# amaas/stanford-ctc

Hardware: AMD Instinct MI355X
Metric: audio frames/sec (CTC fwd-bwd + BRNN grad) at T=1000, L=5, H=1824, |Sigma|=33 (higher is better)
Workload: dtype f32; 1 GPU; WSJ-shape cfg-3: T=1000 A=33 5x1824 BRNN (temporalLayer 3, inputDim 483) U=100, minibatch 32 per GPU, one costAndGrad per step; utterances_per_gpu=32, parallelism=single-gpu

## Files before the change

### stanford-ctc_amd/csrc/recurrent.hip

```cpp
#include <algorithm>
#include <atomic>
#include <map>
#include <mutex>
#include <utility>
#include <vector>

#include <dirent.h>
#include <errno.h>
#include <fcntl.h>
#include <string.h>
#include <string>
#include <type_traits>
#include <sys/stat.h>
#include <sys/file.h>
#include <time.h>
#include <unistd.h>

#include "common.h"
#include "recurrent.h"
#include "xlane.h"

namespace sctc {

typedef void (*RecKernel)(RecArgs);
// ... 365 lines not shown
    const int base = nch >> 2, rem = nch & 3;
    const int cnt = base + (wave < rem ? 1 : 0);
    const int c_beg = wave * base + min(wave, rem);
    float4* Wl = lds4 + (size_t)wave * NLDS * 64;
    float4* red = lds4 + (size_t)4 * NLDS * 64;

    auto load_w = [&](int c) {
        const float* W = p.W[g];
        float4 v;
        if (!p.transpose) {
            v = *reinterpret_cast<const float4*>(W + (int64_t)(row0 + uj) * p.ldw + 16 * c + 4 * kq);
        } else {
            const float* col = W + (int64_t)(16 * c + 4 * kq) * p.ldw + row0 + uj;
            v.x = col[0];
            v.y = col[p.ldw];
            v.z = col[2 * p.ldw];
            v.w = col[3 * p.ldw];
        }
        return v;
    };
    float4 wreg[NREG > 0 ? NREG : 1];
#pragma unroll
    for (int u = 0; u < NREG; ++u) wreg[u] = load_w(c_beg + min(u, cnt - 1));
#pragma unroll 4
    for (int u = NREG; u < NCQ; ++u) Wl[(u - NREG) * 64 + lane] = load_w(c_beg + min(u, cnt - 1));
    __syncthreads();

    const bool desc = p.descending[g] != 0;
    const float* pre = p.pre[g];
    const float* act = p.act[g];
    float* out = p.out[g];
    const int64_t ld = p.ld;
    const float hi = p.max_act > 0.f ? p.max_act : INFINITY;
    unsigned* flags = p.counters + 32 + chain * 128 * REC_FLAG_STRIDE;
    unsigned* err = p.counters + 2;
    const unsigned chunk_stride = (unsigned)p.n_xrows * 64u;
    float* xg = p.xbuf + (size_t)g * p.n_xrows * Hp;
    const __amdgpu_buffer_rsrc_t xrsrc = __builtin_amdgcn_make_buffer_rsrc(
        xg, 0, (int)((size_t)p.n_xrows * Hp * sizeof(float)), 0x00020000);

    const int ub = tile * 16 + uj;
    const int uT = ub < p.B ? p.T_b[ub] : 0;
    const int Tchain = tile * 16 < p.B ? p.T_b[tile * 16] : 0;
    const int tile_T = lane_order_steps(uT, tile, p.b_off, p.variant);

    const int dbg_sel = (p.debug && chain == 0 && tid == 0) ? (wg == 0 ? 0 : (wg == nwg - 1 ? 1 : -1)) : -1;
    auto stamp = [&](int j, int k) {
        if (dbg_sel >= 0 && j >= 64 && j < 80)
            p.debug[(dbg_sel * 16 + (j - 64)) * 8 + k] = (unsigned)clock64();
        if (p.debug && tid == 0 && j == 70) {
            p.debug[REC_DEBUG_ALL_OFF + blockIdx.x * 8 + k] = (unsigned)wall_clock64();
            if (k == 0) p.debug[REC_DEBUG_ALL_OFF + blockIdx.x * 8 + 7] = 1u + (unsigned)chain;
#ifdef SCTC_REC_WHERE
            if (k == 0)
                p.debug[REC_DEBUG_ALL_OFF + blockIdx.x * 8 + 6] =
                    ((__builtin_amdgcn_s_getreg(20 | (0 << 6) | ((4 - 1) << 11)) & 0xf) << 16) |
                    ((__builtin_amdgcn_s_getreg(4 | (0 << 6) | ((32 - 1) << 11)) >> 8) & 0xff);
#endif
        }
    };

    if ((p.variant == 5 && g == 0) || (p.variant == 6 && tile == 0) || (p.variant == 7 && ((g ^ tile) & 1) == 0))
        __builtin_amdgcn_s_setprio(3);
    int rb_next = uT > 0 ? p.rowbase[desc ? uT - 1 : 0] : 0;
    int xb_next = p.xbase[0], xb_cur = 0;
    for (int j = 0; j < Tchain; ++j) {
        stamp(j, 0);
        f32x4 acc[4];
#pragma unroll
        for (int q = 0; q < 4; ++q) acc[q] = {0.f, 0.f, 0.f, 0.f};
        const bool active = j < uT;
        const int xb_prev = xb_cur;
        const int rb = rb_next;
        xb_cur = xb_next;
        {
            const int jn = min(j + 1, Tchain - 1);
            const int tn = desc ? uT - 1 - jn : jn;
            rb_next = p.rowbase[min(max(tn, 0), p.Tmax - 1)];
            xb_next = p.xbase[jn];
        }
        const int64_t orow = active ? (int64_t)rb + p.b_off + ub : 0;
        const unsigned xrow = active ? (unsigned)xb_cur + (unsigned)ub : 0u;
        const unsigned prow = (active && j > 0) ? (unsigned)xb_prev + (unsigned)ub : 0u;
        unsigned xin = prow * 64u + (unsigned)kq * 16u;
        unsigned xout = xrow * 64u + (unsigned)kq * 16u;
        if (j > 0 && j <= tile_T && active) xin = ((unsigned)xb_prev + (unsigned)tile * 16u) * 64u + (unsigned)lane * 16u;
        if (j < tile_T) xout = ((unsigned)xb_cur + (unsigned)tile * 16u) * 64u + (unsigned)lane * 16u;
        float4 pre4 = make_float4(0.f, 0.f, 0.f, 0.f), act4 = pre4;
        if (wave == 0 && active) {
            pre4 = *reinterpret_cast<const float4*>(pre + orow * ld + row0 + 4 * kq);
            if (act) act4 = *reinterpret_cast<const float4*>(act + orow * ld + row0 + 4 * kq);
        }

        if (j > 0) {
            wait_all(flags, nwg, (unsigned)j, err, p.poll_delay);
            stamp(j, 1);
            float4 x[NCQ];
#pragma unroll
            for (int u = 0; u < NCQ; ++u) {
                x[u] = ld_x(xrsrc, xin, (unsigned)(c_beg + min(u, cnt - 1)) * chunk_stride);
                __builtin_amdgcn_sched_barrier(0);
                __builtin_amdgcn_s_sleep(1);
                __builtin_amdgcn_sched_barrier(0);
            }
            __builtin_amdgcn_sched_barrier(0);
#pragma unroll
            for (int u = 0; u < NCQ; ++u) {
                if (u < NCQ - 1 || cnt == NCQ) {
                    const float4 a = u < NREG ? wreg[u < NREG ? u : 0] : Wl[(u - NREG) * 64 + lane];
                    SCTC_MFMA4(acc, a, x[u])
                }
            }
            if (p.debug) {
                asm volatile("" : "+v"(acc[0]), "+v"(acc[1]), "+v"(acc[2]), "+v"(acc[3]));
                stamp(j, 2);
            }
            if (wave != 0) {
                const f32x4 s = (acc[0] + acc[1]) + (acc[2] + acc[3]);
                red[(wave - 1) * 64 + lane] = make_float4(s[0], s[1], s[2], s[3]);
            }
            __syncthreads();
            stamp(j, 3);
        }

        if (wave == 0 && active) {
            float4 s = make_float4(0.f, 0.f, 0.f, 0.f);
            if (j > 0) {
                const float4 r1 = red[lane], r2 = red[64 + lane], r3 = red[128 + lane];
                const f32x4 q = (acc[0] + acc[1]) + (acc[2] + acc[3]);
                s = make_float4((q[0] + r1.x) + (r2.x + r3.x), (q[1] + r1.y) + (r2.y + r3.y),
                                (q[2] + r1.z) + (r2.z + r3.z), (q[3] + r1.w) + (r2.w + r3.w));
            }
            const float4 o = step_result(pre4, s, act4, act != nullptr, hi);
            *reinterpret_cast<float4*>(out + orow * ld + row0 + 4 * kq) = o;
            st_x(xrsrc, xout, (unsigned)wg * chunk_stride, o, sync_mode);
        }
        stamp(j, 4);
        if (j + 1 < Tchain) publish_step(flags + wg * REC_FLAG_STRIDE, (unsigned)(j + 1), sync_mode);
        stamp(j, 5);
    }
}

template <int... I, class F>
__device__ __forceinline__ void static_for_seq(std::integer_sequence<int, I...>, F&& f)
{
    (f(std::integral_constant<int, I>()), ...);
}
template <int N, class F>
__device__ __forceinline__ void static_for(F&& f)
{
    static_for_seq(std::make_integer_sequence<int, N>(), static_cast<F&&>(f));
}

template <int NCQ, int NREGF, int NT, int NBAT, int R, int PUB, int PB>
__global__ __launch_bounds__(256, 1) void brnn_recurrent_t_kernel(RecArgs p)
{
    extern __shared__ __attribute__((aligned(16))) float4 lds4[];
    constexpr int NFR = 2 * NCQ;
    constexpr int NLDSF = NFR - NREGF;
    constexpr int XB = (NCQ + NBAT - 1) / NBAT;
    constexpr int NC = 2 * NT;
    static_assert(NC <= 4, "one result per wave");
    static_assert(NBAT % R == 0 && NBAT >= 2 * R && R >= 2, "ring");
    static_assert((NBAT - 1) * XB < NCQ, "no empty batch");
    static_assert(PUB >= 0 && PUB + 2 <= PB && PB <= NBAT - R + 1 && PB >= 1,
                  "the flag is published (behind batch PUB) before the next phase's flags are polled (in front of batch PB - 1) and "
                  "seen (in front of batch PB), and that before the next phase's first exchange loads (batch NBAT - R + 1)");
    const int tid = threadIdx.x, lane = tid & 63;
    const int wave = __builtin_amdgcn_readfirstlane(tid >> 6);
    const int Hp = p.Hp, nch = Hp >> 4, nprod = Hp >> 5;
    const int combo = blockIdx.x & 3, ublk = blockIdx.x >> 2;
    const int g = combo & 1, half = combo >> 1;
    const int row0 = ublk * 32;
    const int uj = lane & 15, kq = lane >> 4;
    const int sync_mode = p.sync_mode;
    const int base = nch >> 2, rem = nch & 3;
    const int cnt = base + (wave < rem ? 1 : 0);
    const int c_beg = wave * base + min(wave, rem);
    float4* Wl = lds4 + (size_t)wave * NLDSF * 64;
    float4* red = lds4 + (size_t)4 * NLDSF * 64;

    auto load_w = [&](int c, int ug) {
        const float* W = p.W[g];
        const int r = row0 + 16 * ug + uj;
        float4 v;
        if (!p.transpose) {
            v = *reinterpret_cast<const float4*>(W + (int64_t)r * p.ldw + 16 * c + 4 * kq);
        } else {
            const float* col = W + (int64_t)(16 * c + 4 * kq) * p.ldw + r;
            v.x = col[0];
            v.y = col[p.ldw];
            v.z = col[2 * p.ldw];
            v.w = col[3 * p.ldw];
        }
        return v;
    };
    float4 wreg[NREGF > 0 ? NREGF : 1];
    auto load_w0 = [&](int f) {
        const float4 w = load_w(c_beg + min(f >> 1, cnt - 1), f & 1);
        return (f >> 1) < cnt ? w : make_float4(0.f, 0.f, 0.f, 0.f);
    };
#pragma unroll
    for (int f = 0; f < NREGF; ++f) {
        const float4 w = load_w0(f);
        asm("v_accvgpr_write_b32 %0, %1" : "=a"(wreg[f].x) : "v"(w.x));
        asm("v_accvgpr_write_b32 %0, %1" : "=a"(wreg[f].y) : "v"(w.y));
        asm("v_accvgpr_write_b32 %0, %1" : "=a"(wreg[f].z) : "v"(w.z));
        asm("v_accvgpr_write_b32 %0, %1" : "=a"(wreg[f].w) : "v"(w.w));
    }
#pragma unroll 4
    for (int f = NREGF; f < NFR; ++f) Wl[(f - NREGF) * 64 + lane] = load_w0(f);
    __syncthreads();

    const bool desc = p.descending[g] != 0;
    const float* pre = p.pre[g];
    const float* act = p.act[g];
    const float* act_or_pre = act ? act : pre;
    float* out = p.out[g];
    const int64_t ld = p.ld;
    const float hi = p.max_act > 0.f ? p.max_act : INFINITY;
    unsigned* err = p.counters + 2;
    const unsigned chunk_stride = (unsigned)p.n_xrows * 64u;
    float* xg = p.xbuf + (size_t)g * p.n_xrows * Hp;
    const __amdgpu_buffer_rsrc_t xrsrc = __builtin_amdgcn_make_buffer_rsrc(
        xg, 0, (int)((size_t)p.n_xrows * Hp * sizeof(float)), 0x00020000);

    struct Sub {
        int ub[NT], uT[NT], tile_T[NT];
        unsigned trow[NT];
        int T;
        unsigned* flags;
        int rb_next[NT];
        unsigned xb_next, xb_cur;
    };
    auto init_sub = [&](Sub& S, int sub) {
#pragma unroll
        for (int i = 0; i < NT; ++i) {
            const int tile = (i * 2 + sub) * 2 + half;
            S.trow[i] = (unsigned)tile * 16u;
            S.ub[i] = tile * 16 + uj;
            S.uT[i] = S.ub[i] < p.B ? p.T_b[S.ub[i]] : 0;
            S.tile_T[i] = lane_order_steps(S.uT[i], tile, p.b_off, p.variant);
            S.rb_next[i] = S.uT[i] > 0 ? p.rowbase[desc ? S.uT[i] - 1 : 0] : 0;
        }
        S.T = __builtin_amdgcn_readfirstlane((int)S.trow[0] < p.B ? p.T_b[S.trow[0]] : 0);
        S.flags = p.counters + 32 + (size_t)((combo * 2 + sub) * 64) * REC_FLAG_STRIDE;
        S.xb_next = (unsigned)p.xbase[0];
        S.xb_cur = 0;
    };
    int vzero;
    asm volatile("v_mov_b32 %0, 0" : "=v"(vzero));
    Sub A, Bc;
    init_sub(A, 0);
    init_sub(Bc, 1);

    const int dbg_sel = (p.debug && combo == 0 && tid == 0) ? (ublk == 0 ? 0 : (ublk == nprod - 1 ? 1 : -1)) : -1;
    unsigned* dbg_lds = reinterpret_cast<unsigned*>(red + (size_t)2 * NC * 3 * 64);
#if defined(SCTC_T_STAMPS) || defined(SCTC_T_STAMP_CHUNKS)
    auto stamp = [&](int sub, int j, int k) {
        if (dbg_sel >= 0 && j >= 64 && j < 72)
            dbg_lds[((j - 64) * 2 + sub) * 8 + k] = (unsigned)wall_clock64();
    };
#else
    auto stamp = [&](int, int, int) {};
    (void)dbg_lds;
#endif
#ifdef SCTC_T_STAMP_CHUNKS
    unsigned* dbg_fine = dbg_lds + 16 * 8;
    auto stamp_chunk = [&](int sub, int j, int c) {
        if (dbg_sel >= 0 && j >= 64 && j < 68 && c < 32)
            dbg_fine[((j - 64) * 2 + sub) * 32 + c] = (unsigned)wall_clock64();
    };
#else
    auto stamp_chunk = [&](int, int, int) {};
#endif

    float4 x[R][XB][NT];

    auto xin_of = [&](const Sub& S, int j, unsigned xb_prev, unsigned (&xin)[NT]) {
#pragma unroll
        for (int i = 0; i < NT; ++i) {
            const bool active = j < S.uT[i];
            const unsigned prow = (active && j > 0) ? xb_prev + (unsigned)S.ub[i] : 0u;
            xin[i] = prow * 64u + (unsigned)kq * 16u;
            if (j > 0 && j <= S.tile_T[i] && active)
                xin[i] = (xb_prev + S.trow[i]) * 64u + (unsigned)lane * 16u;
            if (p.variant == 49) xin[i] = (unsigned)lane * 16u;
        }
    };
    auto issue_part = [&](const unsigned (&xin)[NT], auto bi_c, auto lo_c, auto hi_c) {
        constexpr int bi = decltype(bi_c)::value, lo = decltype(lo_c)::value, hi_ = decltype(hi_c)::value;
#pragma unroll
        for (int u = lo; u < hi_; ++u) {
            const int cu = bi * XB + u;
            if (cu < NCQ) {
#pragma unroll
                for (int i = 0; i < NT; ++i)
                    x[bi % R][u][i] = ld_x(xrsrc, xin[i], (unsigned)(c_beg + min(cu, cnt - 1)) * chunk_stride);
            }
        }
    };
    auto issue_batch = [&](const unsigned (&xin)[NT], auto bi_c) {
        issue_part(xin, bi_c, std::integral_constant<int, 0>(), std::integral_constant<int, XB>());
    };
    const __amdgpu_buffer_rsrc_t frsrc = __builtin_amdgcn_make_buffer_rsrc(
        p.counters, 0, (int)(REC_COUNTER_WORDS * sizeof(unsigned)), 0x00020000);
    const unsigned flane = (unsigned)min(lane, nprod - 1) * (REC_FLAG_STRIDE * 4u);
    auto flags_off = [&](const unsigned* fl) -> unsigned { return (unsigned)((fl - p.counters) * 4); };
    auto poll_issue = [&](unsigned fl_off) -> u32x4 {
        return __builtin_amdgcn_raw_buffer_load_b128(frsrc, flane, fl_off, 16 );
    };
    auto poll_min = [&](const u32x4& v) -> unsigned {
        unsigned f = v[0];
#pragma unroll
        for (int c = 1; c < NC; ++c) f = min(f, v[c]);
        return f;
    };
    auto wait_flags = [&](unsigned fl_off, unsigned f, unsigned target) {
        if (__all(f >= target)) return;
        const unsigned long long t0 = wall_clock64();
        unsigned spins = 0;
        for (;;) {
            __builtin_amdgcn_s_sleep(1);
            asm volatile("" ::: "memory");
            f = poll_min(poll_issue(fl_off));
            if (__all(f >= target)) break;
            if ((++spins & 255u) == 0) {
                if (spin_expired(err, t0, lane)) break;
            }
        }
    };
    auto prologue = [&](const Sub& S, int j) {
        first_poll_delay(p.poll_delay);
        wait_flags(flags_off(S.flags), poll_min(poll_issue(flags_off(S.flags))), (unsigned)j);
        unsigned xin[NT];
        xin_of(S, j, S.xb_cur, xin);
        static_for<R - 1>([&](auto b) { issue_batch(xin, b); });
    };

    struct Epi {
        bool pending, zero;
        bool lane_active;
        int parity;
        f32x4 mine;
        float4 pre4, act4, r0, r1, r2, s, o;
        int64_t out_off;
        unsigned xo, xchunk;
        unsigned* flag;
        unsigned val;
    };
    Epi E;
    E.pending = false;
    auto epi_barrier = [&](const Epi& e) {
        if (e.pending && !e.zero) {
            asm volatile("s_waitcnt lgkmcnt(0)" ::: "memory");
            __builtin_amdgcn_s_barrier();
            asm volatile("" ::: "memory");
        }
    };
    auto epi_read = [&](Epi& e) {
        if (e.pending && !e.zero && wave < NC) {
            const float4* r = red + (size_t)((e.parity * NC + wave) * 3) * 64 + lane;
            e.r0 = r[0];
            e.r1 = r[64];
            e.r2 = r[128];
        }
    };
    auto epi_sum = [&](Epi& e) {
        e.s = make_float4(0.f, 0.f, 0.f, 0.f);
        if (e.pending && wave < NC && !e.zero) {
            const float4 m = make_float4(e.mine[0], e.mine[1], e.mine[2], e.mine[3]);
            float4 p0 = m, p1 = e.r0, p2 = e.r1, p3 = e.r2;
            if (wave == 1) { p0 = e.r0; p1 = m; }
            if (wave == 2) { p0 = e.r0; p1 = e.r1; p2 = m; }
            if (wave == 3) { p0 = e.r0; p1 = e.r1; p2 = e.r2; p3 = m; }
            e.s = make_float4((p0.x + p1.x) + (p2.x + p3.x), (p0.y + p1.y) + (p2.y + p3.y),
                              (p0.z + p1.z) + (p2.z + p3.z), (p0.w + p1.w) + (p2.w + p3.w));
        }
    };
    auto epi_result = [&](Epi& e) {
        if (e.pending && wave < NC) e.o = step_result(e.pre4, e.s, e.act4, act != nullptr, hi);
    };
    auto epi_stores = [&](const Epi& e) {
        if (e.pending && wave < NC && e.lane_active) {
            *reinterpret_cast<float4*>(out + e.out_off) = e.o;
            st_x(xrsrc, e.xo, e.xchunk, e.o, sync_mode);
        }
    };
    auto epi_store = [&](Epi& e) {
        epi_sum(e);
        epi_result(e);
        epi_stores(e);
    };
    auto epi_publish = [&](Epi& e, auto n_after_c) {
        constexpr int n_after = decltype(n_after_c)::value;
        if (e.pending) {
            if (wave < NC) {
                asm volatile("s_waitcnt vmcnt(%0)" ::"n"(n_after) : "memory");
                if (lane == 0) {
                    if (sync_mode == 0) {
                        __builtin_amdgcn_fence(__ATOMIC_RELEASE, "agent");
                        asm volatile("s_waitcnt vmcnt(0)" ::: "memory");
                    }
                    __hip_atomic_store(e.flag, e.val, __ATOMIC_RELAXED, __HIP_MEMORY_SCOPE_AGENT);
                }
            }
            e.pending = false;
        }
    };
    auto flush = [&](Epi& e) {
        epi_barrier(e);
        epi_read(e);
        epi_store(e);
        epi_publish(e, std::integral_constant<int, 0>());
    };

    int phase_no = 0;
    auto phase = [&](Sub& S, int sub, int j, bool pre_next, const Sub& N, int jn, auto first_c) {
        constexpr bool FIRST = decltype(first_c)::value;
        stamp(sub, j, 0);
        stamp_chunk(sub, j, 0);
        auto late_loads = [&](Epi& en) {
            const int jn2 = min(j + 1, S.T - 1);
            S.xb_next = (unsigned)p.xbase[jn2 + vzero];
#pragma unroll
            for (int i = 0; i < NT; ++i) {
                const int tn = desc ? S.uT[i] - 1 - jn2 : jn2;
                S.rb_next[i] = p.rowbase[min(max(tn, 0), p.Tmax - 1)];
            }
            en.pre4 = *reinterpret_cast<const float4*>(pre + en.out_off);
            en.act4 = *reinterpret_cast<const float4*>(act_or_pre + en.out_off);
        };
        unsigned xin[NT];
        Epi En;
        auto setup = [&]() {
        const unsigned xb_prev = S.xb_cur, xb_cur = S.xb_next;
        S.xb_cur = xb_cur;
        int rb[NT];
#pragma unroll
        for (int i = 0; i < NT; ++i) rb[i] = S.rb_next[i];
        xin_of(S, j, xb_prev, xin);
        En.pending = true;
        En.zero = FIRST;
        En.parity = phase_no & 1;
        En.lane_active = false;
        En.out_off = 0;
        En.xo = 0;
        En.xchunk = (unsigned)(2 * ublk + (wave & 1)) * chunk_stride;
        En.flag = S.flags + ublk * REC_FLAG_STRIDE + wave;
        En.val = (unsigned)(j + 1);
#pragma unroll
        for (int i = 0; i < NT; ++i) {
            if ((wave >> 1) == i && wave < NC) {
                const bool active = j < S.uT[i];
                const int64_t orow = active ? (int64_t)rb[i] + p.b_off + S.ub[i] : 0;
                const unsigned xrow = active ? xb_cur + (unsigned)S.ub[i] : 0u;
                En.xo = xrow * 64u + (unsigned)kq * 16u;
                if (j < S.tile_T[i]) En.xo = (xb_cur + S.trow[i]) * 64u + (unsigned)lane * 16u;
                En.lane_active = active;
                En.out_off = orow * ld + row0 + 16 * (wave & 1) + 4 * kq;
            }
        }
        };
        if constexpr (FIRST) { setup(); late_loads(En); }
        f32x4 acc[2][NT][4];
#pragma unroll
        for (int ug = 0; ug < 2; ++ug)
#pragma unroll
            for (int i = 0; i < NT; ++i)
#pragma unroll
                for (int q = 0; q < 4; ++q) acc[ug][i][q] = {0.f, 0.f, 0.f, 0.f};

        constexpr int WA = 2;
        float4 aq[WA + 1];
        auto prefetch_a = [&](auto G_c) {
            constexpr int G = decltype(G_c)::value, cu = G / NC, f = 2 * cu + ((G % NC) & 1);
            if constexpr (cu < NCQ && f >= NREGF) aq[G % (WA + 1)] = Wl[(f - NREGF) * 64 + lane];
        };
        auto mfma_group = [&](auto bi_c, auto u_c, auto g_c) {
            constexpr int bi = decltype(bi_c)::value, u = decltype(u_c)::value, cu = bi * XB + u;
            constexpr int gi = decltype(g_c)::value >> 1, ug = decltype(g_c)::value & 1;
            constexpr int G = cu * NC + decltype(g_c)::value;
            prefetch_a(std::integral_constant<int, G + WA>());
            if constexpr (cu < NCQ) {
                constexpr int f = 2 * cu + ug;
                float4 a;
                if constexpr (f < NREGF) a = wreg[f]; else a = aq[G % (WA + 1)];
                SCTC_MFMA4(acc[ug][gi], a, x[bi % R][u][gi])
            }
        };
        auto mfma_chunk = [&](auto bi_c, auto u_c) {
            static_for<NC>([&](auto g_c) { mfma_group(bi_c, u_c, g_c); });
        };
        if constexpr (!FIRST) {
            const unsigned nfl_off = flags_off(N.flags);
            u32x4 fl = {0u, 0u, 0u, 0u};
            unsigned xin_n[NT];
#pragma unroll
            for (int i = 0; i < NT; ++i) xin_n[i] = (unsigned)kq * 16u;
            auto issue_one = [&](const unsigned (&xs)[NT], auto bi_c, auto l_c) {
                constexpr int bi = decltype(bi_c)::value, l = decltype(l_c)::value, u = l / NT, i = l % NT, cu = bi * XB + u;
                if constexpr (cu < NCQ)
                    x[bi % R][u][i] = ld_x(xrsrc, xs[i], (unsigned)(c_beg + min(cu, cnt - 1)) * chunk_stride);
            };
            auto park = [&](auto c_c) {
                constexpr int c = decltype(c_c)::value;
                float4* rp = red + (size_t)(En.parity * NC * 3) * 64 + lane;
                const f32x4 s = (acc[c & 1][c >> 1][0] + acc[c & 1][c >> 1][1]) + (acc[c & 1][c >> 1][2] + acc[c & 1][c >> 1][3]);
                if (wave == c) En.mine = s;
                else rp[(c * 3 + (wave < c ? wave : wave - 1)) * 64] = make_float4(s[0], s[1], s[2], s[3]);
            };
            static_for<WA>([&](auto G_c) { prefetch_a(G_c); });
            static_for<NBAT>([&](auto b_c) {
                constexpr int b = decltype(b_c)::value;
                constexpr int nb = b + R - 1;
                constexpr int XBb = (b + 1) * XB <= NCQ ? XB : NCQ - b * XB, NG = XBb * NC;
                constexpr int NL = XB * NT;
#define SCTC_T_SLOT(piece) (NC - 1 + (piece) < NG - 1 ? NC - 1 + (piece) : NG - 1)
                if constexpr (b == PB - 1) {
                    fl = poll_issue(nfl_off);
                    __builtin_amdgcn_sched_barrier(0);
                }
                if constexpr (b == PB) {
                    if (pre_next) {
                        wait_flags(nfl_off, poll_min(fl), (unsigned)jn);
                        xin_of(N, jn, N.xb_cur, xin_n);
                    }
                    __builtin_amdgcn_sched_barrier(0);
                }
                static_for<NG>([&](auto s_c) {
                    constexpr int s = decltype(s_c)::value;
                    mfma_group(b_c, std::integral_constant<int, s / NC>(), std::integral_constant<int, s % NC>());
                    __builtin_amdgcn_sched_barrier(0);
                    if constexpr (b == 0 && s == 0) { setup(); __builtin_amdgcn_sched_barrier(0); }
                    if constexpr (b * XB + s / NC == NCQ - 1 && s % NC >= 1) {
                        park(std::integral_constant<int, s % NC - 1>());
                        __builtin_amdgcn_sched_barrier(0);
                    }
                    if constexpr (s % NC == NC - 1) stamp_chunk(sub, j, 1 + b * XB + s / NC);
                    if constexpr (b == 0) {
                        if constexpr (s % NC == NC - 1 && s / NC < 5) stamp(sub, j, 1 + s / NC);
                        if constexpr (s == SCTC_T_SLOT(0)) { epi_barrier(E); __builtin_amdgcn_sched_barrier(0); }
                        if constexpr (s == SCTC_T_SLOT(1)) { epi_read(E); __builtin_amdgcn_sched_barrier(0); }
                        if constexpr (s == SCTC_T_SLOT(2)) { epi_sum(E); __builtin_amdgcn_sched_barrier(0); }
                        if constexpr (s == SCTC_T_SLOT(3)) { epi_result(E); __builtin_amdgcn_sched_barrier(0); }
                        if constexpr (s == SCTC_T_SLOT(4)) { epi_stores(E); __builtin_amdgcn_sched_barrier(0); }
                    }
                    static_for<NL>([&](auto l_c) {
                        constexpr int l = decltype(l_c)::value, raw = b == 0 ? SCTC_T_SLOT(5) + l : l * NG / NL;
                        if constexpr ((raw < NG - 1 ? raw : NG - 1) == s) {
                            if constexpr (nb < NBAT) issue_one(xin, std::integral_constant<int, nb>(), l_c);
                            else issue_one(xin_n, std::integral_constant<int, nb - NBAT>(), l_c);
                        }
                    });
                    __builtin_amdgcn_sched_barrier(0);
                });
                if constexpr (b == NBAT - 1) {
                    asm volatile("" : "+v"(S.xb_next));
#pragma unroll
                    for (int i = 0; i < NT; ++i) asm volatile("" : "+v"(S.rb_next[i]));
                    asm volatile("" : "+v"(En.pre4.x), "+v"(En.pre4.y), "+v"(En.pre4.z), "+v"(En.pre4.w));
                    asm volatile("" : "+v"(En.act4.x), "+v"(En.act4.y), "+v"(En.act4.z), "+v"(En.act4.w));
                    __builtin_amdgcn_sched_barrier(0);
                }
                if constexpr (b == PUB) {
                    constexpr int first = (R - 1) * XB, end = (R + PUB) * XB < NCQ ? (R + PUB) * XB : NCQ;
                    epi_publish(E, std::integral_constant<int, NT * (end - first)>());
                    __builtin_amdgcn_sched_barrier(0);
                    late_loads(En);
                    __builtin_amdgcn_sched_barrier(0);
                    stamp(sub, j, 6);
                }
            });
            stamp(sub, j, 7);
            park(std::integral_constant<int, NC - 1>());
        } else {
            En.mine = {0.f, 0.f, 0.f, 0.f};
        }
        E = En;
        ++phase_no;
    };

    if (A.T > 0) { phase(A, 0, 0, false, A, 0, std::true_type()); flush(E); }
    if (Bc.T > 0) { phase(Bc, 1, 0, false, Bc, 0, std::true_type()); flush(E); }
    Sub cur = A, nxt = Bc;
    int jc = 1, jn = 1, subc = 0;
    if (jc < cur.T) prologue(cur, jc);
    while (jc < cur.T) {
        const bool pre_next = jn < nxt.T;
        phase(cur, subc, jc, pre_next, nxt, jn, std::false_type());
        ++jc;
        if (pre_next) {
            const Sub t = cur;
            cur = nxt;
            nxt = t;
            const int tj = jc;
            jc = jn;
            jn = tj;
            subc ^= 1;
        } else {
            flush(E);
            if (jc < cur.T) prologue(cur, jc);
        }
    }
#if defined(SCTC_T_STAMPS) || defined(SCTC_T_STAMP_CHUNKS)
    if (dbg_sel >= 0) {
        for (int i = 0; i < 16 * 8; ++i) p.debug[dbg_sel * 16 * 8 + i] = dbg_lds[i];
#ifdef SCTC_T_STAMP_CHUNKS
        for (int i = 0; i < 8 * 32; ++i) p.debug[REC_DEBUG_ALL_OFF + dbg_sel * 8 * 32 + i] = dbg_fine[i];
#endif
    }
#endif
}

#ifdef SCTC_REC_EXPERIMENTS
#include "recurrent_experiments_q8.inc"
#endif

static constexpr unsigned XSENT = 0xffffffffu;

template <int NK, int SB>
__global__ __launch_bounds__(256, 1) void brnn_recurrent_s_kernel(RecArgs p)
{
    extern __shared__ __attribute__((aligned(16))) float4 lds4[];
    float* xs = reinterpret_cast<float*>(lds4);
    const int tid = threadIdx.x, lane = tid & 63;
    const int wave = __builtin_amdgcn_readfirstlane(tid >> 6);
    const int g = blockIdx.x & 1, wg = blockIdx.x >> 1;
    const int Hp = p.Hp;
    const int rg = tid >> 5, ks = tid & 31;
    const int row0 = wg * 16 + 2 * rg;
    const bool owner = ks == 31;

    float w0[NK], w1[NK];
    {
        const float* W = p.W[g];
#pragma unroll
        for (int i = 0; i < NK; ++i) {
            const int k = 32 * i + ks;
            if (!p.transpose) {
                w0[i] = W[(int64_t)row0 * p.ldw + k];
                w1[i] = W[(int64_t)(row0 + 1) * p.ldw + k];
            } else {
                w0[i] = W[(int64_t)k * p.ldw + row0];
                w1[i] = W[(int64_t)k * p.ldw + row0 + 1];
            }
        }
    }
    const bool desc = p.descending[g] != 0;
    const float* pre = p.pre[g];
    const float* act = p.act[g];
    float* out = p.out[g];
    const int64_t ld = p.ld;
    const float hi = p.max_act > 0.f ? p.max_act : INFINITY;
    unsigned* err = p.counters + 2;
    float* xg = p.xbuf + (size_t)g * p.n_xrows * Hp;
    const __amdgpu_buffer_rsrc_t xrsrc = __builtin_amdgcn_make_buffer_rsrc(
        xg, 0, (int)((size_t)p.n_xrows * Hp * sizeof(float)), 0x00020000);
    int Tb[SB];
#pragma unroll
    for (int b = 0; b < SB; ++b) Tb[b] = b < p.B ? p.T_b[b] : 0;
// ... 668 lines not shown

static int read_error_word(const RecArgs& a, hipStream_t stream, unsigned* e)
{
    *e = 0;
    SCTC_HIP_TRY(hipMemcpyAsync(e, a.counters + 2, sizeof(unsigned), hipMemcpyDeviceToHost, stream));
    SCTC_HIP_TRY(hipStreamSynchronize(stream));
    return SCTC_OK;
}

static int launch_persistent(RecKernel k, int grid, size_t smem, int max_per_cu, size_t sentinel_bytes,
                             const RecArgs& a, const LaunchCtx& cx, bool* done, int threads = 256)
{
    *done = false;
    int per_cu = 0;
    SCTC_TRY(prepare_kernel(k, threads, smem, max_per_cu, cx.dev, &per_cu));
    if (per_cu < 1 || (int64_t)per_cu * cx.cus < grid) return SCTC_OK;
    const int need_cus = (grid + per_cu - 1) / per_cu;
    if (sentinel_bytes)
        SCTC_HIP_TRY(hipMemsetAsync(a.xbuf, 0xFF, sentinel_bytes, cx.stream));
    if (!recurrent_shared_device_mode() && !g_shared_hard.load(std::memory_order_relaxed) && g_users.due(cx.dev)) {
        const int n = g_users.count(cx.dev);
        if (n > 1) {
            recurrent_set_shared_device_mode(1);
            fprintf(stderr, "sctc: %d processes run persistent kernels on this GPU: shared-device mode on "
                            "(their launches take turns under /dev/shm/sctc_gpu_*.lock)\n", n);
        }
    }
    if (recurrent_shared_device_mode()) {
        SCTC_HIP_TRY(hipStreamSynchronize(cx.stream));
        LeaseGuard lease(cx.dev);
        if (!lease.locked) return SCTC_OK;
        hipLaunchKernelGGL(k, dim3(grid), dim3(threads), smem, cx.stream, a);
        SCTC_HIP_TRY(hipGetLastError());
        unsigned e = 0;
        SCTC_TRY(read_error_word(a, cx.stream, &e));
        *done = true;
        if (cx.path) *cx.path = REC_PATH_PERSISTENT_LEASED;
        if (e != 0)
            return set_error(SCTC_ERR_TIMEOUT, "recurrent kernel: a persistent launch under the device lease gave "
                             "up waiting for its peers (%d workgroups not co-resident)", grid);
        return SCTC_OK;
    }
    SCTC_TRY(g_gate.admit_and_launch(cx.dev, cx.stream, need_cus, cx.cus, [&]() {
        hipLaunchKernelGGL(k, dim3(grid), dim3(threads), smem, cx.stream, a);
        return hipGetLastError();
    }));
    *done = true;
    if (cx.path) *cx.path = REC_PATH_PERSISTENT;
    return SCTC_OK;
}

static int launch_recurrent_one(const RecArgs& a, const LaunchCtx& cx)
{
    const int nwg = a.Hp / 16;
    const int ntiles = (a.B + 15) / 16;
    hipStream_t stream = cx.stream;
    bool done = false;
    SCTC_HIP_TRY(hipMemsetAsync(a.counters + 32, 0, (REC_COUNTER_WORDS - 32) * sizeof(unsigned), stream));
    if (a.variant == 3 || 2 * nwg > cx.cus) {
        if (cx.path) *cx.path = REC_PATH_FALLBACK;
        return launch_fallback(a, stream);
    }
    if ((!a.prec16 || a.B <= 5) && (a.B > Q1_MIN_B - 1 || a.variant == 44) && a.B <= 16 && a.variant != 1 && a.variant != 42 && a.variant != 43 &&
        2 * nwg <= cx.cus) {
        RecKernel qk = nullptr;
        int ncq = 0, nreg = 0;
        switch (nwg) {
            case 32:  qk = brnn_recurrent_q_kernel<8, 0>;   ncq = 8;  nreg = 0;  break;
            case 64:  qk = brnn_recurrent_q_kernel<16, 0>;  ncq = 16; nreg = 0;  break;
            case 114: qk = brnn_recurrent_q_kernel<29, 10>; ncq = 29; nreg = 10; break;
            case 128: qk = brnn_recurrent_q_kernel<32, 13>; ncq = 32; nreg = 13; break;
            default: break;
        }
        if (qk) {
            RecArgs b = a;
            b.linear_map = 1;
            if (b.variant == 44) b.variant = 0;
            const size_t smem = sizeof(float4) * ((size_t)4 * (ncq - nreg) * 64 + 3 * 64);
            SCTC_TRY(launch_persistent(qk, 2 * nwg, smem, 2, 0, b, cx, &done));
            if (done) return SCTC_OK;
        }
    }
    if ((a.B <= 5 || (a.B <= 8 && a.variant == 43)) && a.variant != 1) {
        RecKernel sk = nullptr;
        const bool s4 = a.B <= 4;
        switch (a.Hp / 32) {
            case 16: sk = s4 ? brnn_recurrent_s_kernel<16, 4> : brnn_recurrent_s_kernel<16, 8>; break;
            case 32: sk = s4 ? brnn_recurrent_s_kernel<32, 4> : brnn_recurrent_s_kernel<32, 8>; break;
            case 57: sk = s4 ? brnn_recurrent_s_kernel<57, 4> : brnn_recurrent_s_kernel<57, 8>; break;
            case 64: sk = s4 ? brnn_recurrent_s_kernel<64, 4> : brnn_recurrent_s_kernel<64, 8>; break;
            default: break;
        }
        if (sk) {
            const size_t smem = sizeof(float) * 2 * (s4 ? 4 : 8) * a.Hp;
            SCTC_TRY(launch_persistent(sk, 2 * nwg, smem, 2, (size_t)2 * a.n_xrows * a.Hp * sizeof(float), a, cx, &done));
            if (done) return SCTC_OK;
        }
    }
    if (a.prec16 && a.B > 5 && a.B <= 16 && a.variant != 1) {
        RecKernel hk = nullptr;
        const bool bf = a.transpose != 0;
        const int nch = a.Hp / 32;
        switch ((nch + 3) / 4) {
            case 4:  if (nch == 16) hk = bf ? brnn_recurrent_mh_kernel<4, true>  : brnn_recurrent_mh_kernel<4, false>;  break;
            case 8:  if (nch == 32) hk = bf ? brnn_recurrent_mh_kernel<8, true>  : brnn_recurrent_mh_kernel<8, false>;  break;
            case 15: if (nch == 57) hk = bf ? brnn_recurrent_mh_kernel<15, true> : brnn_recurrent_mh_kernel<15, false>; break;
            case 16: if (nch == 64) hk = bf ? brnn_recurrent_mh_kernel<16, true> : brnn_recurrent_mh_kernel<16, false>; break;
            default: break;
        }
        const size_t smem = (((size_t)16 * (a.Hp + 8) * 2 + 15) / 16) * 16 + 3 * 64 * sizeof(float4);
        if (hk && smem <= 160 * 1024) {
            SCTC_TRY(launch_persistent(hk, 2 * nwg, smem, 1, (size_t)2 * a.n_xrows * a.Hp * 2, a, cx, &done));
            if (done) return SCTC_OK;
        }
    }
#ifdef SCTC_REC_EXPERIMENTS
    if (a.B > 5 && a.B <= 16 && a.variant != 1) {
        RecKernel mk = nullptr;
        switch ((nwg + 3) / 4) {
            case 8:  if (nwg == 32)  mk = brnn_recurrent_m_kernel<8>;  break;
            case 16: if (nwg == 64)  mk = brnn_recurrent_m_kernel<16>; break;
            case 29: if (nwg == 114) mk = brnn_recurrent_m_kernel<29>; break;
            case 32: if (nwg == 128) mk = brnn_recurrent_m_kernel<32>; break;
            default: break;
        }
        const size_t smem = sizeof(float) * ((size_t)16 * (a.Hp + 4) + 3 * 256);
        if (mk && smem <= 160 * 1024) {
            SCTC_TRY(launch_persistent(mk, 2 * nwg, smem, 1, (size_t)2 * a.n_xrows * a.Hp * sizeof(float), a, cx, &done));
            if (done) return SCTC_OK;
        }
    }
#endif
#ifdef SCTC_REC_EXPERIMENTS
    const int q8_variant = (a.variant >= 8 && a.variant < 40) ? a.variant : (a.variant == 0 ? REC_Q8_DEFAULT : 0);
    if (ntiles == 2 && q8_variant >= 8) {
        RecKernel k8 = nullptr;
        switch (nwg) {
            case 32:  k8 = brnn_recurrent_q8_kernel<8>;  break;
            case 64:  k8 = brnn_recurrent_q8_kernel<16>; break;
            case 114: k8 = brnn_recurrent_q8_kernel<29>; break;
            case 128: k8 = brnn_recurrent_q8_kernel<32>; break;
            default: break;
        }
        const int grid = 8 * ((nwg + 3) / 4);
        const size_t smem = sizeof(float4) * ((size_t)nwg * 64 + 6 * 64) + sizeof(unsigned) * Q8_SYNC_WORDS;
        if (k8 && grid <= cx.cus && smem <= 160 * 1024) {
            RecArgs b = a;
            b.variant = q8_variant;
            SCTC_TRY(launch_persistent(k8, grid, smem, 1, 0, b, cx, &done, 512));
            if (done) return SCTC_OK;
        }
    }
#endif
    if (ntiles == 2 && a.variant != 1 && 4 * nwg <= 2 * cx.cus && (4 * nwg) % 8 == 0) {
        RecKernel qk = nullptr;
        int ncq = 0, nreg = 0;
        switch (nwg) {
            case 32:  qk = brnn_recurrent_q_kernel<8, 0>;   ncq = 8;  nreg = 0;  break;
            case 64:  qk = brnn_recurrent_q_kernel<16, 0>;  ncq = 16; nreg = 0;  break;
            case 114: qk = brnn_recurrent_q_kernel<29, 10>; ncq = 29; nreg = 10; break;
            case 128: qk = brnn_recurrent_q_kernel<32, 13>; ncq = 32; nreg = 13; break;
            default: break;
        }
        if (qk) {
            const size_t smem = sizeof(float4) * ((size_t)4 * (ncq - nreg) * 64 + 3 * 64);
            SCTC_TRY(launch_persistent(qk, 4 * nwg, smem, 2, 0, a, cx, &done));
            if (done) return SCTC_OK;
        }
    }
    if (ntiles > 2 && a.variant != 1 && a.variant != 40 && a.variant != 47 && 4 * (a.Hp / 32) <= cx.cus &&
        (a.Hp >= 1824 || a.variant == 50)) {
        RecKernel tk = nullptr;
        const bool one = ntiles <= 4;
        int nldsf = 0;
        static const int tcfg = getenv("SCTC_REC_TCFG") ? atoi(getenv("SCTC_REC_TCFG")) : 0;
        switch (nwg) {
            case 32:  tk = one ? brnn_recurrent_t_kernel<8, 0, 1, 4, 2, 0, 3>  : brnn_recurrent_t_kernel<8, 0, 2, 4, 2, 0, 3>;  nldsf = 16; break;
            case 64:  tk = one ? brnn_recurrent_t_kernel<16, 0, 1, 4, 2, 1, 3> : brnn_recurrent_t_kernel<16, 0, 2, 4, 2, 1, 3>; nldsf = 32; break;
            case 114:
                nldsf = 33;
                if (one) tk = tcfg == 1 ? brnn_recurrent_t_kernel<29, 25, 1, 6, 3, 1, 4> : tcfg == 2 ? brnn_recurrent_t_kernel<29, 25, 1, 8, 2, 1, 7>
                              : brnn_recurrent_t_kernel<29, 25, 1, 8, 4, 1, 5>;
                else tk = tcfg == 1 ? brnn_recurrent_t_kernel<29, 25, 2, 8, 4, 1, 5> : tcfg == 2 ? brnn_recurrent_t_kernel<29, 25, 2, 8, 2, 1, 7>
                          : brnn_recurrent_t_kernel<29, 25, 2, 6, 3, 1, 4>;
                break;
            case 128:
                nldsf = 33;
                if (one) tk = tcfg == 1 ? brnn_recurrent_t_kernel<32, 31, 1, 6, 3, 1, 4> : brnn_recurrent_t_kernel<32, 31, 1, 8, 4, 1, 5>;
                else tk = tcfg == 1 ? brnn_recurrent_t_kernel<32, 31, 2, 6, 3, 1, 4> : brnn_recurrent_t_kernel<32, 31, 2, 8, 4, 1, 5>;
                break;
            default: break;
        }
        if (tk) {
            const size_t smem = sizeof(float4) * 64 * ((size_t)4 * nldsf + 2 * 3 * (one ? 2 : 4)) + (16 * 8 + 8 * 32) * sizeof(unsigned);
            SCTC_TRY(launch_persistent(tk, 4 * (a.Hp / 32), smem, 1, 0, a, cx, &done));
            if (done) return SCTC_OK;
        }
    }
    const int ntw = ntiles <= 2 ? 1 : (ntiles <= 4 ? 2 : 4);
    const size_t smem = sizeof(float4) * ((size_t)nwg * 64 + 2 * ntw * 64);
    if (smem <= 160 * 1024) {
        const bool pipe = a.variant != 40;
        RecKernel kern = ntw == 1 ? pick_kernel<1>(nwg / 2, false)
                         : (ntw == 2 ? pick_kernel<2>(nwg / 2, pipe) : pick_kernel<4>(nwg / 2, pipe));
        SCTC_TRY(launch_persistent(kern, 2 * nwg, smem, 1, 0, a, cx, &done));
        if (done) return SCTC_OK;
    }
    if (cx.path) *cx.path = REC_PATH_FALLBACK;
    return launch_fallback(a, stream);
}

int recurrent_clear_error(unsigned* counters, hipStream_t stream)
{
    SCTC_HIP_TRY(hipMemsetAsync(counters, 0, 32 * sizeof(unsigned), stream));
    return SCTC_OK;
}

int launch_recurrent(const RecArgs& a_in, hipStream_t stream, int* path)
{
    RecArgs a = a_in;
    if (a.poll_delay < 0) a.poll_delay = a.Hp > 1024 ? 5 : 0;
    char why[128];
    if (!recurrent_supported(a.Hp, a.B, why, sizeof(why)))
        return set_error(SCTC_ERR_ARG, "recurrent kernel: %s", why);
    if (a.Tmax <= 0 || a.B <= 0) return SCTC_OK;
    if ((size_t)a.n_xrows * a.Hp * sizeof(float) >= ((size_t)1 << 31))
        return set_error(SCTC_ERR_ARG, "recurrent kernel: %d exchange rows x %d units exceed the "
                         "2 GiB buffer addressing", a.n_xrows, a.Hp);
    LaunchCtx cx;
    cx.stream = stream;
    cx.path = path;
    cx.dev = 0;
    cx.cus = 0;
    SCTC_HIP_TRY(hipGetDevice(&cx.dev));
    SCTC_HIP_TRY(hipDeviceGetAttribute(&cx.cus, hipDeviceAttributeMultiprocessorCount, cx.dev));
    constexpr int MAXB = 128;
    for (int b0 = 0; b0 < a_in.B;) {
        int nb = std::min(MAXB, a_in.B - b0);
        const bool tiled = ((a.variant == 0 && (a.Hp == 1824 || a.Hp == 2048)) || (a.variant == 50 && (a.Hp == 512 || a.Hp == 1024 || a.Hp == 1824 || a.Hp == 2048))) &&
                           !a.prec16 && 4 * (a.Hp / 32) <= cx.cus;
        if (tiled) {
            if (nb > 64 && nb <= 96) nb = 64;
        } else {
            if (nb > 32 && nb <= 48 && a.variant == 0 && !a.prec16) nb = 32;
            else if (nb > 64 && nb <= 80 && a.variant == 0 && !a.prec16) nb = 64;
        }
        RecArgs c = a;
        c.b_off = a_in.b_off + b0;
        c.T_b = a_in.T_b + b0;
        c.B = nb;
        if (a_in.T_host) c.Tmax = std::min(a_in.Tmax, (int)a_in.T_host[b0]);
        if (c.variant == 45) c.variant = 0;
        SCTC_TRY(launch_recurrent_one(c, cx));
        b0 += nb;
    }
    return SCTC_OK;
}

}
```

Measured before the change: 763,400 frames/s.

## Add 16-unit-per-block variant of transposed recurrent kernel for two-tile case

Generalizes the transposed recurrent kernel with a UG parameter so each workgroup can own 16 hidden units instead of 32. This doubles the number of producer blocks, widens the flag polling to two flags per lane, and remaps flag slots for blocks beyond 64. A new dispatch path for the two-tile fp32 case launches this variant ahead of the older q kernel, with all weights held in registers by default. The aim is to spread the serial recurrence over more CUs and cut per-block matmul work per step, at the cost of more cross-block synchronisation and flag traffic per timestep.

```diff
diff --git a/stanford-ctc_amd/csrc/recurrent.hip b/stanford-ctc_amd/csrc/recurrent.hip
--- a/stanford-ctc_amd/csrc/recurrent.hip
+++ b/stanford-ctc_amd/csrc/recurrent.hip
@@ -541,15 +541,17 @@
     static_for_seq(std::make_integer_sequence<int, N>(), static_cast<F&&>(f));
 }
 
-template <int NCQ, int NREGF, int NT, int NBAT, int R, int PUB, int PB>
+template <int NCQ, int NREGF, int NT, int NBAT, int R, int PUB, int PB, int UG = 2>
 __global__ __launch_bounds__(256, 1) void brnn_recurrent_t_kernel(RecArgs p)
 {
     extern __shared__ __attribute__((aligned(16))) float4 lds4[];
-    constexpr int NFR = 2 * NCQ;
+    constexpr int NFR = UG * NCQ;
     constexpr int NLDSF = NFR - NREGF;
     constexpr int XB = (NCQ + NBAT - 1) / NBAT;
-    constexpr int NC = 2 * NT;
-    static_assert(NC <= 4, "one result per wave");
+    constexpr int NC = UG * NT;
+    constexpr int NPL = UG == 1 ? 2 : 1;
+    static_assert(UG == 1 || UG == 2, "16 or 32 units per block");
+    static_assert(NC <= 4 && NPL * NC <= 4, "one result per wave, one 16-byte flag load per lane");
     static_assert(NBAT % R == 0 && NBAT >= 2 * R && R >= 2, "ring");
     static_assert((NBAT - 1) * XB < NCQ, "no empty batch");
     static_assert(PUB >= 0 && PUB + 2 <= PB && PB <= NBAT - R + 1 && PB >= 1,
@@ -557,10 +559,10 @@
                   "seen (in front of batch PB), and that before the next phase's first exchange loads (batch NBAT - R + 1)");
     const int tid = threadIdx.x, lane = tid & 63;
     const int wave = __builtin_amdgcn_readfirstlane(tid >> 6);
-    const int Hp = p.Hp, nch = Hp >> 4, nprod = Hp >> 5;
-    const int combo = blockIdx.x & 3, ublk = blockIdx.x >> 2;
+    const int Hp = p.Hp, nch = Hp >> 4, nprod = nch / UG;
+    const int combo = blockIdx.x & (2 * UG - 1), ublk = blockIdx.x / (2 * UG);
     const int g = combo & 1, half = combo >> 1;
-    const int row0 = ublk * 32;
+    const int row0 = ublk * 16 * UG;
     const int uj = lane & 15, kq = lane >> 4;
     const int sync_mode = p.sync_mode;
     const int base = nch >> 2, rem = nch & 3;
@@ -586,8 +588,8 @@
     };
     float4 wreg[NREGF > 0 ? NREGF : 1];
     auto load_w0 = [&](int f) {
-        const float4 w = load_w(c_beg + min(f >> 1, cnt - 1), f & 1);
-        return (f >> 1) < cnt ? w : make_float4(0.f, 0.f, 0.f, 0.f);
+        const float4 w = load_w(c_beg + min(f / UG, cnt - 1), f % UG);
+        return (f / UG) < cnt ? w : make_float4(0.f, 0.f, 0.f, 0.f);
     };
 #pragma unroll
     for (int f = 0; f < NREGF; ++f) {
@@ -625,7 +627,7 @@
     auto init_sub = [&](Sub& S, int sub) {
 #pragma unroll
         for (int i = 0; i < NT; ++i) {
-            const int tile = (i * 2 + sub) * 2 + half;
+            const int tile = (i * 2 + sub) * UG + half;
             S.trow[i] = (unsigned)tile * 16u;
             S.ub[i] = tile * 16 + uj;
             S.uT[i] = S.ub[i] < p.B ? p.T_b[S.ub[i]] : 0;
@@ -703,6 +705,11 @@
         unsigned f = v[0];
 #pragma unroll
         for (int c = 1; c < NC; ++c) f = min(f, v[c]);
+        if constexpr (NPL == 2) {
+            const bool second = lane + 64 < nprod;
+#pragma unroll
+            for (int c = 0; c < NC; ++c) f = second ? min(f, v[NC + c]) : f;
+        }
         return f;
     };
     auto wait_flags = [&](unsigned fl_off, unsigned f, unsigned target) {
@@ -835,26 +842,26 @@
         En.lane_active = false;
         En.out_off = 0;
         En.xo = 0;
-        En.xchunk = (unsigned)(2 * ublk + (wave & 1)) * chunk_stride;
-        En.flag = S.flags + ublk * REC_FLAG_STRIDE + wave;
+        En.xchunk = (unsigned)(UG * ublk + wave % UG) * chunk_stride;
+        En.flag = S.flags + (ublk & 63) * REC_FLAG_STRIDE + (ublk >> 6) * NC + wave;
         En.val = (unsigned)(j + 1);
 #pragma unroll
         for (int i = 0; i < NT; ++i) {
-            if ((wave >> 1) == i && wave < NC) {
+            if (wave / UG == i && wave < NC) {
                 const bool active = j < S.uT[i];
                 const int64_t orow = active ? (int64_t)rb[i] + p.b_off + S.ub[i] : 0;
                 const unsigned xrow = active ? xb_cur + (unsigned)S.ub[i] : 0u;
                 En.xo = xrow * 64u + (unsigned)kq * 16u;
                 if (j < S.tile_T[i]) En.xo = (xb_cur + S.trow[i]) * 64u + (unsigned)lane * 16u;
                 En.lane_active = active;
-                En.out_off = orow * ld + row0 + 16 * (wave & 1) + 4 * kq;
+                En.out_off = orow * ld + row0 + 16 * (wave % UG) + 4 * kq;
             }
         }
         };
         if constexpr (FIRST) { setup(); late_loads(En); }
-        f32x4 acc[2][NT][4];
-#pragma unroll
-        for (int ug = 0; ug < 2; ++ug)
+        f32x4 acc[UG][NT][4];
+#pragma unroll
+        for (int ug = 0; ug < UG; ++ug)
 #pragma unroll
             for (int i = 0; i < NT; ++i)
 #pragma unroll
@@ -863,16 +870,16 @@
         constexpr int WA = 2;
         float4 aq[WA + 1];
         auto prefetch_a = [&](auto G_c) {
-            constexpr int G = decltype(G_c)::value, cu = G / NC, f = 2 * cu + ((G % NC) & 1);
+            constexpr int G = decltype(G_c)::value, cu = G / NC, f = UG * cu + (G % NC) % UG;
             if constexpr (cu < NCQ && f >= NREGF) aq[G % (WA + 1)] = Wl[(f - NREGF) * 64 + lane];
         };
         auto mfma_group = [&](auto bi_c, auto u_c, auto g_c) {
             constexpr int bi = decltype(bi_c)::value, u = decltype(u_c)::value, cu = bi * XB + u;
-            constexpr int gi = decltype(g_c)::value >> 1, ug = decltype(g_c)::value & 1;
+            constexpr int gi = decltype(g_c)::value / UG, ug = decltype(g_c)::value % UG;
             constexpr int G = cu * NC + decltype(g_c)::value;
             prefetch_a(std::integral_constant<int, G + WA>());
             if constexpr (cu < NCQ) {
-                constexpr int f = 2 * cu + ug;
+                constexpr int f = UG * cu + ug;
                 float4 a;
                 if constexpr (f < NREGF) a = wreg[f]; else a = aq[G % (WA + 1)];
                 SCTC_MFMA4(acc[ug][gi], a, x[bi % R][u][gi])
@@ -895,7 +902,7 @@
             auto park = [&](auto c_c) {
                 constexpr int c = decltype(c_c)::value;
                 float4* rp = red + (size_t)(En.parity * NC * 3) * 64 + lane;
-                const f32x4 s = (acc[c & 1][c >> 1][0] + acc[c & 1][c >> 1][1]) + (acc[c & 1][c >> 1][2] + acc[c & 1][c >> 1][3]);
+                const f32x4 s = (acc[c % UG][c / UG][0] + acc[c % UG][c / UG][1]) + (acc[c % UG][c / UG][2] + acc[c % UG][c / UG][3]);
                 if (wave == c) En.mine = s;
                 else rp[(c * 3 + (wave < c ? wave : wave - 1)) * 64] = make_float4(s[0], s[1], s[2], s[3]);
             };
@@ -1870,6 +1877,30 @@
         }
     }
 #endif
+    if (ntiles == 2 && !a.prec16 && (a.variant == 0 || a.variant == 46 || a.variant == 49) && 2 * nwg <= cx.cus) {
+        static const int tcfg = getenv("SCTC_REC_TCFG") ? atoi(getenv("SCTC_REC_TCFG")) : 0;
+        RecKernel tk = nullptr;
+        int nldsf = 0;
+        switch (nwg) {
+            case 114:
+                tk = tcfg == 1 ? brnn_recurrent_t_kernel<29, 29, 1, 6, 3, 1, 4, 1> : tcfg == 3 ? brnn_recurrent_t_kernel<29, 0, 1, 8, 4, 1, 5, 1>
+                     : brnn_recurrent_t_kernel<29, 29, 1, 8, 4, 1, 5, 1>;
+                nldsf = tcfg == 3 ? 29 : 0;
+                break;
+            case 128:
+                tk = tcfg == 1 ? brnn_recurrent_t_kernel<32, 32, 1, 6, 3, 1, 4, 1> : tcfg == 3 ? brnn_recurrent_t_kernel<32, 0, 1, 8, 4, 1, 5, 1>
+                     : brnn_recurrent_t_kernel<32, 32, 1, 8, 4, 1, 5, 1>;
+                nldsf = tcfg == 3 ? 32 : 0;
+                break;
+            default: break;
+        }
+        if (tk) {
+            size_t smem = sizeof(float4) * 64 * ((size_t)4 * nldsf + 2 * 3 * 1) + (16 * 8 + 8 * 32) * sizeof(unsigned);
+            smem = std::max(smem, (size_t)81 * 1024);
+            SCTC_TRY(launch_persistent(tk, 2 * nwg, smem, 1, 0, a, cx, &done));
+            if (done) return SCTC_OK;
+        }
+    }
     if (ntiles == 2 && a.variant != 1 && 4 * nwg <= 2 * cx.cus && (4 * nwg) % 8 == 0) {
         RecKernel qk = nullptr;
         int ncq = 0, nreg = 0;
```

Result: faster. 819,400 frames/s (median of 6 runs) (+7.3%).
